# eridgd/WCT-TF

Hardware: NVIDIA B200
Metric: 512x512 5-level WCT stylised frames/sec (higher is better)
Workload: dtype f32

## Files before the change

wct_tf_b200/_capi.py:

```python
from __future__ import annotations

import ctypes as C
import os

_HERE = os.path.dirname(os.path.abspath(__file__))
LIB_PATH = os.path.join(_HERE, "libwctb200.so")

RELU = 1
CLIP01 = 2
HALO_EDGE = 4
POOL2 = 8
EINVAL, ECUDA, EWS, EDEVICE = -1, -2, -3, -4

_vp, _i, _f, _sz = C.c_void_p, C.c_int, C.c_float, C.c_size_t

SIGNATURES = {
    "wctb200_abi_version": (_i, []),
    "wctb200_last_error": (C.c_char_p, []),
    "wctb200_check_device": (_i, [_vp]),
    "wctb200_act_bytes": (_sz, [_i, _i, _i, _i]),
    "wctb200_act_from_f32": (_i, [_vp, _i, _i, _i, _i, _vp, _vp]),
    "wctb200_act_to_f32": (_i, [_vp, _i, _i, _i, _i, _vp, _vp]),
    "wctb200_image_u8_to_f32": (_i, [_vp, _sz, _vp, _vp]),
    "wctb200_image_f32_to_u8": (_i, [_vp, _sz, _vp, _vp]),
    "wctb200_resize_workspace_bytes": (_sz, [_i, _i, _i, _i, _i, _i, _i]),
    "wctb200_resize_bilinear_u8": (_i, [_vp, _i, _i, _i, _i, _i, _i, _i, _i, _i, _i, _vp, _vp, _sz, _vp]),
    "wctb200_rgb_moments_u8": (_i, [_vp, C.c_longlong, _vp, _vp]),
    "wctb200_coral_apply_u8": (_i, [_vp, C.c_longlong, _vp, _vp, _vp, _vp, _vp, _vp, _vp]),
    "wctb200_conv_weight_bytes": (_sz, [_i, _i, _i]),
    "wctb200_prep_conv_weights": (_i, [_vp, _i, _i, _i, _vp, _vp]),
    "wctb200_prep_conv_weights_up2": (_i, [_vp, _i, _i, _vp, _vp]),
    "wctb200_conv3x3": (_i, [_vp, _i, _i, _i, _i, _vp, _vp, _i, _i, _vp, _vp]),
    "wctb200_conv3x3_up2": (_i, [_vp, _i, _i, _i, _i, _vp, _vp, _i, _i, _vp, _vp]),
    "wctb200_conv3x3_ref": (_i, [_vp, _i, _i, _i, _i, _vp, _vp, _i, _i, _vp, _vp]),
    "wctb200_conv_head": (_i, [_vp, _i, _i, _i, _vp, _vp, _vp, _vp]),
    "wctb200_conv_tail": (_i, [_vp, _i, _i, _i, _i, _vp, _vp, _i, _vp, _vp]),
    "wctb200_maxpool2": (_i, [_vp, _i, _i, _i, _i, _vp, _vp]),
    "wctb200_upsample2": (_i, [_vp, _i, _i, _i, _i, _vp, _vp]),
    "wctb200_wct_workspace_bytes": (_sz, [_i, _i, _i]),
    "wctb200_wct_level": (_i, [_vp, _i, _i, _i, _vp, _i, _i, _i, _i, _f, _f, _f, _f, _i, _vp, _vp, _vp, _sz, _vp]),
    "wctb200_wct_style_state_bytes": (_sz, [_i, _i]),
    "wctb200_wct_style_prepare": (_i, [_vp, _i, _i, _i, _i, _f, _f, _f, _vp, _vp, _sz, _vp]),
    "wctb200_wct_apply": (_i, [_vp, _i, _i, _i, _i, _vp, _i, _f, _f, _f, _f, _i, _vp, _vp, _vp, _sz, _vp]),
    "wctb200_adain_level": (_i, [_vp, _i, _i, _i, _vp, _i, _i, _i, _i, _f, _f, _vp, _vp, _sz, _vp]),
    "wctb200_covariance": (_i, [_vp, _i, _i, _i, _i, _f, _vp, _vp, _vp]),
    "wctb200_jacobi_eigh": (_i, [_vp, _i, _i, _vp, _vp, _vp]),
    "wctb200_style_swap_workspace_bytes": (_sz, [_i, _i, _i, _i, _i, _i, _i]),
    "wctb200_style_swap_level": (_i, [_vp, _i, _i, _vp, _i, _i, _i, _i, _i, _f, _f, _f, _vp, _vp, _vp, _sz, _vp]),
}

DEBUG_SIGNATURES = {
    "wctb200_debug_set_conv_bn": (_i, [_i]),
    "wctb200_debug_set_conv_oversub": (_i, [_i]),
    "wctb200_debug_set_conv_fuse": (_i, [_i]),
    "wctb200_debug_set_jacobi": (_i, [_i, _i]),
    "wctb200_debug_set_jacobi_tolq": (_i, [_f]),
    "wctb200_debug_set_conv_products": (_i, [_i]),
    "wctb200_debug_set_conv_tail_tc": (_i, [_i]),
    "wctb200_debug_set_conv_head_tc": (_i, [_i]),
    "wctb200_debug_set_matfun": (_i, [_i, _i]),
    "wctb200_debug_matfun": (_i, [_vp, _i, _i, _i, _f, _f, _vp, _vp, _vp, _vp]),
    "wctb200_debug_set_cov_stages": (_i, [_i]),
}

_lib = None


class WctB200Error(RuntimeError):
    pass


def load():
    global _lib
    if _lib is not None:
        return _lib
    if not os.path.exists(LIB_PATH):
        raise WctB200Error("%s not found: build it with `python -c 'import __graft_entry__ as g; g.build()'` "
                           "(there is no CPU fallback)" % LIB_PATH)
    lib = C.CDLL(LIB_PATH)
    for table in (SIGNATURES, DEBUG_SIGNATURES):
        for name, (res, args) in table.items():
            fn = getattr(lib, name)
            fn.restype = res
            fn.argtypes = args
    if lib.wctb200_abi_version() != 1:
        raise WctB200Error("libwctb200 ABI version mismatch")
    _lib = lib
    return lib


def check(rc):
    if rc != 0:
        raise WctB200Error("libwctb200 error %d: %s" % (rc, load().wctb200_last_error().decode()))
```

wct_tf_b200/csrc/capi.cu:

```cuda
#include <stdarg.h>
#include <string.h>

#include <map>
#include <mutex>
#include <tuple>

#include "common.cuh"
#include "wctb200_debug.h"

namespace wctb {

static thread_local char t_err[512] = "";

void set_error(const char* fmt, ...) {
    va_list ap;
    va_start(ap, fmt);
    vsnprintf(t_err, sizeof(t_err), fmt, ap);
    va_end(ap);
}
int cuda_fail(cudaError_t e, const char* what) {
    set_error("CUDA error %d (%s) at %s", (int)e, cudaGetErrorString(e), what);
    return WCTB200_ECUDA;
}

// ... 6 lines not shown
    std::lock_guard<std::mutex> lock(mu);
    Entry& e = cache[std::make_tuple(dev, st, slot)];
    if (e.cap < bytes) {
        if (e.p) {
            WCTB_CUDA(cudaStreamSynchronize(st));
            WCTB_CUDA(cudaFree(e.p));
            e.p = nullptr;
            e.cap = 0;
        }
        const size_t cap = bytes + bytes / 8 + 256;
        WCTB_CUDA(cudaMalloc(&e.p, cap));
        e.cap = cap;
    }
    *ptr = e.p;
    return 0;
}

__device__ unsigned int g_device_error = 0;

unsigned int* device_error_word() {
    static unsigned int* ptr[64] = {nullptr};
    int dev = 0;
    cudaGetDevice(&dev);
    if (dev < 0 || dev >= 64) dev = 0;
    if (!ptr[dev]) {
        void* p = nullptr;
        if (cudaGetSymbolAddress(&p, g_device_error) == cudaSuccess) ptr[dev] = static_cast<unsigned int*>(p);
    }
    return ptr[dev];
}

int device_sm_count() {
    static std::atomic<int> sms[64];
    int dev = 0;
    cudaGetDevice(&dev);
    dev &= 63;
    int v = sms[dev].load(std::memory_order_relaxed);
    if (v <= 0) {
        if (cudaDeviceGetAttribute(&v, cudaDevAttrMultiProcessorCount, dev) != cudaSuccess || v <= 0) v = 148;
        sms[dev].store(v, std::memory_order_relaxed);
    }
    return v;
}

int launch_u8_to_f32(const uint8_t*, size_t, float*, cudaStream_t);
int launch_f32_to_u8(const float*, size_t, uint8_t*, cudaStream_t);
size_t resize_workspace_bytes(int N, int Hs, int Ws, int C, int Hd, int Wd, int Wout);
int launch_resize_u8(const uint8_t* src, int N, int Hs, int Ws, int C, int Hd, int Wd, int y0, int x0, int Hout, int Wout,
                     uint8_t* dst, void* ws, size_t ws_bytes, cudaStream_t st);
int launch_rgb_moments(const uint8_t* img, long long npix, unsigned long long* sums, cudaStream_t st);
int launch_coral_apply(const uint8_t* src, long long npix, const double* A, const double* sm, const double* ss, const double* tm,
                       const double* ts, uint8_t* dst, cudaStream_t st);
int launch_act_from_f32(const float*, ActGeom, __half*, cudaStream_t);
int launch_act_to_f32(const __half*, ActGeom, float*, cudaStream_t);
int launch_prep_weights(const float*, int, int, int, __half*, cudaStream_t);
int launch_prep_weights_up2(const float*, int, int, __half*, cudaStream_t);
size_t style_swap_workspace_bytes(int C, int Hc, int Wc, int Hs, int Ws, int P, int S);
int launch_style_swap_level(const __half* content, int Hc, int Wc, const __half* style, int Hs, int Ws, int C, int patch, int stride,
                            float alpha, float eps_cov, float thresh, __half* out, int32_t* k_out, void* ws, size_t ws_bytes,
                            cudaStream_t st);
int launch_conv3x3_ref(const __half*, ActGeom, const float*, const float*, int, int, __half*, cudaStream_t);
int launch_conv_head(const float*, int, int, int, const float*, const float*, __half*, cudaStream_t);
int launch_conv_tail(const __half*, ActGeom, const float*, const float*, int, float*, cudaStream_t);
int launch_maxpool2(const __half*, ActGeom, __half*, cudaStream_t);
int launch_upsample2(const __half*, ActGeom, __half*, cudaStream_t);
size_t wct_workspace_bytes(int, int, int);
int launch_wct_level(const __half*, int, int, int, const __half*, int, int, int, int, float, float, float, float, int,
                     __half*, int32_t*, void*, size_t, cudaStream_t);
int launch_adain_level(const __half*, int, int, int, const __half*, int, int, int, int, float, float, __half*, void*,
                       size_t, cudaStream_t);
size_t wct_style_state_bytes(int, int);
int launch_wct_style_prepare(const __half*, int, int, int, int, float, float, float, void*, void*, size_t, cudaStream_t);
int launch_wct_apply(const __half*, int, int, int, int, const void*, int, float, float, float, float, int, __half*, int32_t*,
                     void*, size_t, cudaStream_t);
int launch_covariance(const __half*, int, int, int, int, float, float*, float*, cudaStream_t);
int launch_jacobi(float*, int, int, float*, int*, cudaStream_t, const int* skip);
int launch_eig_post(const float*, const float*, float*, int, int, float, float, int, float*, float*, int*, cudaStream_t, const int* skip);
extern int g_conv_bn_override;
extern int g_conv_oversub;
extern int g_conv_fuse;
extern int g_conv_products;
extern int g_conv_tail_tc;
extern int g_conv_head_tc;
int launch_matfun_ns(const float* A, int C, int count, int n_first, float thresh, float eps_eig, float* out, int* ok, int* kcount,
                     cudaStream_t st, float* info);
extern int g_matfun;
extern int g_matfun_max_it;
extern int g_cov_max_stages;
int set_jacobi_tolq(float v);
extern int g_jacobi_lg;
extern int g_jacobi_stagger;

static bool geom_ok(int N, int H, int W, int C) {
    return N >= 1 && H >= 2 && W >= 2 && C >= 8 && C % 8 == 0 &&
           (long long)N * (2ll * H + 2) * (2ll * W + 2) * (C / 8) < (1ll << 32) && (long long)H * W < (1ll << 31);
}

}

using namespace wctb;

#define ST(s) static_cast<cudaStream_t>(s)
#define HP(p) static_cast<__half*>(p)
#define HCP(p) static_cast<const __half*>(p)

extern "C" {

int wctb200_abi_version(void) { return WCTB200_ABI_VERSION; }
const char* wctb200_last_error(void) { return t_err; }

int wctb200_check_device(void* stream) {
    WCTB_CUDA(cudaStreamSynchronize(ST(stream)));
    unsigned int* w = device_error_word();
    if (!w) {
        set_error("device error word unavailable (no CUDA device?)");
        return WCTB200_ECUDA;
    }
    unsigned int v = 0;
    WCTB_CUDA(cudaMemcpy(&v, w, sizeof(v), cudaMemcpyDeviceToHost));
    if (v != 0) {
        unsigned int zero = 0;
        cudaMemcpy(w, &zero, sizeof(zero), cudaMemcpyHostToDevice);
        set_error("device-side pipeline time-out, code 0x%x (0x1xx producer wait, 0x2xx MMA wait, 0x3xx epilogue wait)", v);
        return WCTB200_EDEVICE;
    }
    return 0;
}

size_t wctb200_act_bytes(int N, int H, int W, int C) {
    if (!geom_ok(N, H, W, C)) return 0;
    ActGeom g(N, H, W, C);
    return (size_t)g.plane * 2 * sizeof(__half);
}

int wctb200_act_from_f32(const float* nhwc, int N, int H, int W, int C, void* act, void* stream) {
    WCTB_REQUIRE(geom_ok(N, H, W, C) && nhwc && act, "act_from_f32: bad arguments");
    return launch_act_from_f32(nhwc, ActGeom(N, H, W, C), HP(act), ST(stream));
}
int wctb200_act_to_f32(const void* act, int N, int H, int W, int C, float* nhwc, void* stream) {
    WCTB_REQUIRE(geom_ok(N, H, W, C) && nhwc && act, "act_to_f32: bad arguments");
    return launch_act_to_f32(HCP(act), ActGeom(N, H, W, C), nhwc, ST(stream));
}

int wctb200_image_u8_to_f32(const uint8_t* img, size_t count, float* out, void* stream) {
    WCTB_REQUIRE(img && out, "image_u8_to_f32: null pointer");
    if (count == 0) return 0;
    return launch_u8_to_f32(img, count, out, ST(stream));
}
int wctb200_image_f32_to_u8(const float* img, size_t count, uint8_t* out, void* stream) {
    WCTB_REQUIRE(img && out, "image_f32_to_u8: null pointer");
    if (count == 0) return 0;
    return launch_f32_to_u8(img, count, out, ST(stream));
}

static bool resize_args_ok(int N, int Hs, int Ws, int C, int Hd, int Wd) {
    return N >= 1 && Hs >= 1 && Ws >= 1 && C >= 1 && C <= 4 && Hd >= 1 && Wd >= 1 && Hs <= (1 << 15) && Ws <= (1 << 15) &&
           Hd <= (1 << 15) && Wd <= (1 << 15);
}
size_t wctb200_resize_workspace_bytes(int N, int Hs, int Ws, int C, int Hd, int Wd, int Wout) {
    if (!resize_args_ok(N, Hs, Ws, C, Hd, Wd) || Wout < 1 || Wout > Wd) return 0;
    return resize_workspace_bytes(N, Hs, Ws, C, Hd, Wd, Wout);
}
int wctb200_resize_bilinear_u8(const uint8_t* src, int N, int Hs, int Ws, int C, int Hd, int Wd, int y0, int x0, int Hout,
                               int Wout, uint8_t* dst, void* ws, size_t ws_bytes, void* stream) {
    WCTB_REQUIRE(src && dst && ws, "resize_bilinear_u8: null pointer");
    WCTB_REQUIRE(resize_args_ok(N, Hs, Ws, C, Hd, Wd), "resize_bilinear_u8: bad geometry N=%d %dx%dx%d -> %dx%d", N, Hs, Ws, C, Hd, Wd);
// ... 90 lines not shown
                      void* ws, size_t ws_bytes, void* stream) {
    WCTB_REQUIRE(content && state && out && ws, "wct_apply: null pointer");
    WCTB_REQUIRE(geom_ok(Nc, Hc, Wc, C), "wct_apply: bad geometry");
    return launch_wct_apply(HCP(content), Nc, Hc, Wc, C, state, Ns, alpha, eps_cov, eps_eig, thresh, readd_content_mean,
                            HP(out), k_out, ws, ws_bytes, ST(stream));
}
int wctb200_adain_level(const void* content, int Nc, int Hc, int Wc, const void* style, int Ns, int Hs, int Ws, int C,
                        float alpha, float eps, void* out, void* ws, size_t ws_bytes, void* stream) {
    WCTB_REQUIRE(content && style && out && ws, "adain_level: null pointer");
    WCTB_REQUIRE(geom_ok(Nc, Hc, Wc, C) && geom_ok(Ns, Hs, Ws, C), "adain_level: bad geometry");
    return launch_adain_level(HCP(content), Nc, Hc, Wc, HCP(style), Ns, Hs, Ws, C, alpha, eps, HP(out), ws, ws_bytes,
                              ST(stream));
}

int wctb200_covariance(const void* act, int N, int H, int W, int C, float eps_cov, float* mean, float* cov, void* stream) {
    WCTB_REQUIRE(act && mean && cov && geom_ok(N, H, W, C), "covariance: bad arguments");
    return launch_covariance(HCP(act), N, H, W, C, eps_cov, mean, cov, ST(stream));
}

int wctb200_jacobi_eigh(float* a, int C, int count, float* sigma, int32_t* sweeps, void* stream) {
    WCTB_REQUIRE(a && sigma && count >= 1, "jacobi_eigh: bad arguments");
    WCTB_REQUIRE(C == 64 || C == 128 || C == 256 || C == 512, "jacobi_eigh: C=%d not in {64,128,256,512}", C);
    const size_t nmat = (size_t)count * C * C;
    float* scratch = nullptr;
    {
        int rc0 = scratch_alloc(reinterpret_cast<void**>(&scratch), ((size_t)count * 16 + nmat + (size_t)count * C) * sizeof(float), ST(stream), 2);
        if (rc0) return rc0;
    }
    float* conv = scratch;
    float* a0 = scratch + (size_t)count * 16;
    float* lam = a0 + nmat;
    cudaError_t ce = cudaMemcpyAsync(a0, a, nmat * sizeof(float), cudaMemcpyDeviceToDevice, ST(stream));
    int rc = ce == cudaSuccess ? launch_jacobi(a, C, count, conv, sweeps, ST(stream), nullptr) : cuda_fail(ce, "cudaMemcpyAsync");
    if (!rc) rc = launch_eig_post(a, a0, lam, C, count, 0.f, 0.f, count, sigma, nullptr, nullptr, ST(stream), nullptr);
    return rc;
}

size_t wctb200_style_swap_workspace_bytes(int C, int Hc, int Wc, int Hs, int Ws, int patch, int stride) {
    if (!geom_ok(1, Hc, Wc, C) || !geom_ok(1, Hs, Ws, C) || patch < 1 || patch > 16 || stride < 1 || stride > 16 || Hc < patch ||
        Wc < patch || Hs < patch || Ws < patch)
        return 0;
    return style_swap_workspace_bytes(C, Hc, Wc, Hs, Ws, patch, stride);
}
int wctb200_style_swap_level(const void* content, int Hc, int Wc, const void* style, int Hs, int Ws, int C, int patch, int stride,
                             float alpha, float eps_cov, float thresh, void* out, int32_t* k_out, void* ws, size_t ws_bytes,
                             void* stream) {
    WCTB_REQUIRE(content && style && out && ws, "style_swap_level: null pointer");
    WCTB_REQUIRE(geom_ok(1, Hc, Wc, C) && geom_ok(1, Hs, Ws, C), "style_swap_level: bad geometry");
    return launch_style_swap_level(HCP(content), Hc, Wc, HCP(style), Hs, Ws, C, patch, stride, alpha, eps_cov, thresh, HP(out), k_out, ws,
                                   ws_bytes, ST(stream));
}
int wctb200_debug_set_conv_bn(int bn) {
    g_conv_bn_override = bn;
    return 0;
}
int wctb200_debug_set_conv_oversub(int k) {
    g_conv_oversub = k < 1 ? 1 : (k > 16 ? 16 : k);
    return g_conv_oversub;
}
int wctb200_debug_set_conv_fuse(int mode) {
    g_conv_fuse = mode < 0 ? -1 : (mode ? 1 : 0);
    return g_conv_fuse;
}
int wctb200_debug_set_jacobi_tolq(float tolq) { return set_jacobi_tolq(tolq); }
int wctb200_debug_set_cov_stages(int n) {
    if (n >= 1 && n <= 12) g_cov_max_stages = n;
    return g_cov_max_stages;
}
int wctb200_debug_matfun(const float* A, int C, int count, int n_first, float thresh, float eps_eig, float* out, int* ok,
                         float* info, void* stream) {
    WCTB_REQUIRE(A && out && ok && count >= 1 && n_first >= 0 && n_first <= count, "debug_matfun: bad arguments");
    const int rc = launch_matfun_ns(A, C, count, n_first, thresh, eps_eig, out, ok, nullptr, ST(stream), info);
    return rc < 0 ? rc : 0;
}
int wctb200_debug_set_matfun(int mode, int max_it) {
    if (mode == 0 || mode == 1) g_matfun = mode;
    if (max_it >= 1 && max_it <= 64) g_matfun_max_it = max_it;
    return g_matfun;
}
int wctb200_debug_set_conv_head_tc(int on) {
    if (on == 0 || on == 1) g_conv_head_tc = on;
    return g_conv_head_tc;
}
int wctb200_debug_set_conv_tail_tc(int on) {
    if (on == 0 || on == 1) g_conv_tail_tc = on;
    return g_conv_tail_tc;
}
int wctb200_debug_set_conv_products(int n) {
    if (n >= 1 && n <= 3) g_conv_products = n;
    return g_conv_products;
}

int wctb200_debug_set_jacobi(int lg_groups, int stagger_cycles) {
    if (lg_groups <= 4) g_jacobi_lg = lg_groups < 0 ? -1 : lg_groups;
    g_jacobi_stagger = stagger_cycles < 0 ? -1 : stagger_cycles;
    return g_jacobi_lg;
}

}
```

wct_tf_b200/csrc/common.cuh:

```cuda
#pragma once

#include <cuda.h>
#include <cuda_fp16.h>
#include <cuda_runtime.h>
#include <stdint.h>
#include <stdio.h>

#include <atomic>

#include "../../include/wctb200.h"

namespace wctb {

void set_error(const char* fmt, ...);
int cuda_fail(cudaError_t e, const char* what);
unsigned int* device_error_word();

#define WCTB_CUDA(call)                                        \
    do {                                                       \
        cudaError_t _e = (call);                               \
        if (_e != cudaSuccess) return ::wctb::cuda_fail(_e, #call); \
    } while (0)

#define WCTB_CHECK_LAUNCH(name)                                \
// ... 203 lines not shown
__device__ __forceinline__ bool mbar_try_wait(uint64_t* bar, uint32_t parity) {
    uint32_t ok;
    asm volatile(
        "{\n\t.reg .pred p;\n\t"
#ifdef WCTB_MBAR_TEST_WAIT
        "mbarrier.test_wait.parity.shared::cta.b64 p, [%1], %2;\n\t"
#else
        "mbarrier.try_wait.parity.shared::cta.b64 p, [%1], %2;\n\t"
#endif
        "selp.u32 %0, 1, 0, p;\n\t}"
        : "=r"(ok)
        : "r"(smem_u32(bar)), "r"(parity)
        : "memory");
    return ok != 0;
}
__device__ __forceinline__ unsigned long long globaltimer_ns() {
    unsigned long long t;
    asm volatile("mov.u64 %0, %globaltimer;" : "=l"(t));
    return t;
}
__device__ __forceinline__ void mbar_wait(uint64_t* bar, uint32_t parity, volatile int* abort_flag,
                                          unsigned int* err_word, unsigned int code) {
    if (mbar_try_wait(bar, parity)) return;
    const long long t0 = clock64();
    for (unsigned int it = 1;; ++it) {
        if (mbar_try_wait(bar, parity)) return;
        if ((it & 255u) == 0u) {
            if (*abort_flag) return;
            if (*reinterpret_cast<volatile unsigned int*>(err_word)) { *abort_flag = 1; return; }
            if (clock64() - t0 > 4000000000ll) break;
        }
    }
    *abort_flag = 1;
    atomicExch(err_word, code);
}

__device__ __forceinline__ void tma_prefetch_desc(const void* map) {
    asm volatile("prefetch.tensormap [%0];" ::"l"(reinterpret_cast<uint64_t>(map)) : "memory");
}
__device__ __forceinline__ void tma_load_3d(void* smem_dst, const void* map, uint64_t* bar, int c0, int c1, int c2) {
    asm volatile(
        "cp.async.bulk.tensor.3d.shared::cluster.global.mbarrier::complete_tx::bytes [%0], [%1, {%3, %4, %5}], [%2];"
        ::"r"(smem_u32(smem_dst)), "l"(reinterpret_cast<uint64_t>(map)), "r"(smem_u32(bar)), "r"(c0), "r"(c1), "r"(c2)
        : "memory");
}

__device__ __forceinline__ void tc_fence_before() { asm volatile("tcgen05.fence::before_thread_sync;" ::: "memory"); }
__device__ __forceinline__ void tc_fence_after() { asm volatile("tcgen05.fence::after_thread_sync;" ::: "memory"); }

__device__ __forceinline__ void tmem_alloc(uint32_t* smem_slot, uint32_t ncols) {
    asm volatile("tcgen05.alloc.cta_group::1.sync.aligned.shared::cta.b32 [%0], %1;" ::"r"(smem_u32(smem_slot)), "r"(ncols)
                 : "memory");
    asm volatile("tcgen05.relinquish_alloc_permit.cta_group::1.sync.aligned;" ::: "memory");
}
__device__ __forceinline__ void tmem_dealloc(uint32_t taddr, uint32_t ncols) {
    asm volatile("tcgen05.dealloc.cta_group::1.sync.aligned.b32 %0, %1;" ::"r"(taddr), "r"(ncols) : "memory");
}
__device__ __forceinline__ void umma_f16(uint32_t tmem_d, uint64_t desc_a, uint64_t desc_b, uint32_t idesc,
                                         uint32_t accumulate) {
    asm volatile(
        "{\n\t.reg .pred p;\n\t"
        "setp.ne.b32 p, %4, 0;\n\t"
        "tcgen05.mma.cta_group::1.kind::f16 [%0], %1, %2, %3, p;\n\t}"
        ::"r"(tmem_d), "l"(desc_a), "l"(desc_b), "r"(idesc), "r"(accumulate)
        : "memory");
}
__device__ __forceinline__ void umma_commit(uint64_t* bar) {
    asm volatile("tcgen05.commit.cta_group::1.mbarrier::arrive::one.shared::cluster.b64 [%0];" ::"r"(smem_u32(bar))
                 : "memory");
}
__device__ __forceinline__ void tmem_ld32(uint32_t taddr, uint32_t* r) {
    asm volatile(
        "tcgen05.ld.sync.aligned.32x32b.x32.b32 "
        "{%0, %1, %2, %3, %4, %5, %6, %7, %8, %9, %10, %11, %12, %13, %14, %15, "
        "%16, %17, %18, %19, %20, %21, %22, %23, %24, %25, %26, %27, %28, %29, %30, %31}, [%32];"
        : "=r"(r[0]), "=r"(r[1]), "=r"(r[2]), "=r"(r[3]), "=r"(r[4]), "=r"(r[5]), "=r"(r[6]), "=r"(r[7]), "=r"(r[8]),
          "=r"(r[9]), "=r"(r[10]), "=r"(r[11]), "=r"(r[12]), "=r"(r[13]), "=r"(r[14]), "=r"(r[15]), "=r"(r[16]),
          "=r"(r[17]), "=r"(r[18]), "=r"(r[19]), "=r"(r[20]), "=r"(r[21]), "=r"(r[22]), "=r"(r[23]), "=r"(r[24]),
          "=r"(r[25]), "=r"(r[26]), "=r"(r[27]), "=r"(r[28]), "=r"(r[29]), "=r"(r[30]), "=r"(r[31])
        : "r"(taddr)
        : "memory");
}
__device__ __forceinline__ void tmem_ld_wait() { asm volatile("tcgen05.wait::ld.sync.aligned;" ::: "memory"); }

__device__ __forceinline__ uint64_t umma_desc_sw128(uint32_t smem_addr) {
    uint64_t d = 0;
    d |= (uint64_t)((smem_addr >> 4) & 0x3FFF);
    d |= (uint64_t)1 << 16;
    d |= (uint64_t)(1024 >> 4) << 32;
    d |= (uint64_t)1 << 46;
    d |= (uint64_t)2 << 61;
    return d;
}
__host__ __device__ constexpr uint32_t umma_idesc_f16(int M, int N) {
    return (1u << 4)
           | (0u << 7) | (0u << 10)
           | (0u << 15) | (0u << 16)
           | ((uint32_t)(N >> 3) << 17)
           | ((uint32_t)(M >> 4) << 24);
}
__device__ __forceinline__ uint64_t umma_desc_mn_sw128(uint32_t smem_addr) {
    uint64_t d = 0;
    d |= (uint64_t)((smem_addr >> 4) & 0x3FFF);
    d |= (uint64_t)((8192 >> 4) & 0x3FFF) << 16;
    d |= (uint64_t)((1024 >> 4) & 0x3FFF) << 32;
    d |= (uint64_t)1 << 46;
    d |= (uint64_t)2 << 61;
    return d;
}
__host__ __device__ constexpr uint32_t umma_idesc_f16_mn(int M, int N) {
    return (1u << 4) | (1u << 15) | (1u << 16) | ((uint32_t)(N >> 3) << 17) | ((uint32_t)(M >> 4) << 24);
}
__device__ __forceinline__ void tmem_ld16(uint32_t taddr, uint32_t* r) {
    asm volatile(
        "tcgen05.ld.sync.aligned.32x32b.x16.b32 "
        "{%0, %1, %2, %3, %4, %5, %6, %7, %8, %9, %10, %11, %12, %13, %14, %15}, [%16];"
        : "=r"(r[0]), "=r"(r[1]), "=r"(r[2]), "=r"(r[3]), "=r"(r[4]), "=r"(r[5]), "=r"(r[6]), "=r"(r[7]), "=r"(r[8]),
          "=r"(r[9]), "=r"(r[10]), "=r"(r[11]), "=r"(r[12]), "=r"(r[13]), "=r"(r[14]), "=r"(r[15])
        : "r"(taddr)
        : "memory");
}
#endif

int scratch_alloc(void** ptr, size_t bytes, cudaStream_t st, int slot);

enum ConvMode { CONV_3X3 = 0, CONV_APPLY = 1, CONV_UP2 = 2, CONV_TAPS = 3 };
int launch_conv_tc(int mode, const __half* in, int N, int H, int W, int Cin, const __half* w_split, int nsets,
                   const float* wscale, const float* bias, int Cout, int flags, __half* out, cudaStream_t st, int kw = 3);
static inline const float* weight_scale_ptr(const __half* w_split, int taps_total, int Cin, int Cout) {
    return reinterpret_cast<const float*>(w_split + (size_t)2 * taps_total * Cin * Cout);
}

}
```

wct_tf_b200/csrc/conv_tc.cu:

```cuda
#include "common.cuh"

namespace wctb {

extern int g_conv_bn_override;

struct ConvParams {
    int N, H, W, Cin, Cout, Hp, Wp;
    long long P;
    int mode;
    int taps;
    int kw;
    int products;
    int per_image;
    int pool;
    int pool_tx, pool_ho;
    int nsets;
    int tiles_per_image;
    int flags;
    const float* bias;
    const float* wscale;
    __half* out;
    unsigned int* err;
};

template <int BN, bool FUSE_>
struct Conv2Cfg {
    static constexpr int BM = 128;
    static constexpr int BK = 64;
    static constexpr int A_BYTES = BM * BK * 2;
    static constexpr int B_BYTES = BN * BK * 2;
    static constexpr int STAGE_BYTES = 2 * A_BYTES + 2 * B_BYTES;
    static constexpr int STAGES = BN == 64 ? 4 : (BN == 128 ? 3 : 2);
    static constexpr bool FUSE = FUSE_ && BN <= 128;
    static constexpr int ACC_COLS = FUSE ? 2 * BN : BN;
    static constexpr int NBUF = 512 / ACC_COLS >= 4 ? 4 : 2;
    static constexpr int TMEM_COLS = NBUF * ACC_COLS;
    static constexpr int CH = 4;
    static constexpr int EPI_WARPS = BN == 256 ? 8 : 4;
    static constexpr int THREADS = 64 + 32 * EPI_WARPS;
    static constexpr int NACC = BN / (EPI_WARPS / 4);
    static constexpr int AUX_BYTES = 256 + BN * 4;
    static constexpr int STG_BYTES = BN <= 128 ? 4 * 8192 : 0;
    static constexpr int SMEM_BYTES = STAGES * STAGE_BYTES + AUX_BYTES + STG_BYTES + 1024;
};

struct TileCoord {
    long long p0, p_end;
    int n0, set;
    int cls;
};

__device__ __forceinline__ TileCoord tile_coord(const ConvParams& p, int tile, int n_tiles, int BN) {
    TileCoord t;
    const int nt = tile % n_tiles;
    int mt = tile / n_tiles;
    const long long HpWp = (long long)p.Hp * p.Wp;
    t.n0 = nt * BN;
    t.cls = 0;
    if (p.pool) {
        const int t_ = mt % p.pool_tx;
        const int r_ = mt / p.pool_tx;
        const int i_ = r_ % p.pool_ho;
        const int img = r_ / p.pool_ho;
        t.p0 = img * HpWp + (long long)(2 * i_ + 1) * p.Wp + 1 + 64 * t_;
        t.p_end = p.P;
        t.set = 0;
        t.cls = t_;
    } else if (p.mode == CONV_UP2) {
        t.cls = mt & 3;
        mt >>= 2;
        t.p0 = (long long)mt * 128;
        t.p_end = p.P;
        t.set = t.cls;
    } else if (p.per_image) {
        const int img = mt / p.tiles_per_image;
        const int r = mt - img * p.tiles_per_image;
        t.p0 = img * HpWp + (long long)r * 128;
        t.p_end = (img + 1) * HpWp;
        t.set = p.nsets > 1 ? img : 0;
    } else {
        t.p0 = (long long)mt * 128;
        t.p_end = p.P;
        t.set = 0;
    }
    return t;
}

template <int BN, bool FUSE_>
__global__ void __launch_bounds__(Conv2Cfg<BN, FUSE_>::THREADS, 1)
conv_tc2_kernel(const __grid_constant__ CUtensorMap mapA, const __grid_constant__ CUtensorMap mapB,
                const __grid_constant__ CUtensorMap mapA64, const ConvParams p, const int total_tiles, const int n_tiles) {
    using Cfg = Conv2Cfg<BN, FUSE_>;
    extern __shared__ uint8_t smem_raw[];
    uint8_t* smem = smem_raw + ((1024u - (smem_u32(smem_raw) & 1023u)) & 1023u);
    uint8_t* aux = smem + Cfg::STAGES * Cfg::STAGE_BYTES;
    uint64_t* full = reinterpret_cast<uint64_t*>(aux);
    uint64_t* empty = full + Cfg::STAGES;
    uint64_t* tfull = empty + Cfg::STAGES;
    uint64_t* tempty = tfull + Cfg::NBUF;
    uint32_t* tmem_slot = reinterpret_cast<uint32_t*>(tempty + Cfg::NBUF);
// ... 190 lines not shown
#pragma unroll
                    for (int h = 0; h < 2; ++h) {
                        const float a0 = acc[h * NH + c0], a1 = acc[h * NH + c0 + 8];
                        const float mine = lp ? a1 : a0;
                        const float other = lp ? a0 : a1;
                        mh[h] = fmaxf(mine, __shfl_xor_sync(0xffffffffu, other, 1));
                    }
                    keep[k] = hv ? mh[1] : mh[0];
                    send[k] = hv ? mh[0] : mh[1];
                }
                uint8_t* stg_all = aux + Cfg::AUX_BYTES;
                {
                    float* xb = reinterpret_cast<float*>(stg_all + e * 8192) + lane;
#pragma unroll
                    for (int k = 0; k < Q; ++k) xb[k * 32] = send[k];
                }
                asm volatile("bar.sync 1, %0;" ::"r"(ETHREADS) : "memory");
                {
                    const float* pb = reinterpret_cast<const float*>(stg_all + (e ^ 2) * 8192) + lane;
#pragma unroll
                    for (int k = 0; k < Q; ++k) keep[k] = fmaxf(keep[k], pb[k * 32]);
                }
                const int xe = x & ~1;
                if (xe < p.W && yy0 - 1 < p.H && !*abort_flag) {
                    const int yo = (yy0 - 1) >> 1, xo = xe >> 1;
                    const int flags = halo_flags(go, yo, xo);
                    const unsigned int ppos = (n * (unsigned int)go.Hp + (unsigned int)(yo + 1)) * (unsigned int)go.Wp + (unsigned int)(xo + 1);
                    const int cb = colbase + hv * NH + lp * 8;
#pragma unroll
                    for (int q = 0; q < Q / 8; ++q) {
                        float v[8];
#pragma unroll
                        for (int j = 0; j < 8; ++j) {
                            const float t = fmaf(keep[q * 8 + j], wsc, sbias[cb + q * 16 + j]);
                            v[j] = relu ? fmaxf(t, 0.f) : t;
                        }
                        Half8 hi, lo;
                        split8(v, hi, lo);
                        store8_at(p.out, go, ppos, flags, tc.n0 + cb + q * 16, hi, lo);
                    }
                }
                continue;
            }
            const unsigned int pos = (unsigned int)tc.p0 + (unsigned int)(g * 32 + lane);
            int flags = -1;
            unsigned int ppos = 0;
            if (pos < (unsigned int)tc.p_end) {
                const unsigned int hpwp = (unsigned int)(p.Hp * p.Wp);
                const unsigned int n = pos / hpwp;
                const unsigned int r = pos - n * hpwp;
                const int yy = (int)(r / (unsigned int)p.Wp);
                const int xx = (int)(r - (unsigned int)yy * (unsigned int)p.Wp);
                if (yy >= 1 && yy <= p.H && xx >= 1 && xx <= p.W && !*abort_flag) {
                    int y = yy - 1, x = xx - 1;
                    if (up2) { y = 2 * y + (tc.cls >> 1); x = 2 * x + (tc.cls & 1); }
                    flags = halo_flags(go, y, x);
                    ppos = ((unsigned int)n * (unsigned int)go.Hp + (unsigned int)(y + 1)) * (unsigned int)go.Wp + (unsigned int)(x + 1);
                }
            }
            if (Cfg::STG_BYTES > 0) {
                uint8_t* stg = aux + Cfg::AUX_BYTES + e * 8192;
                store_tile_rows<Cfg::NACC>(acc, wsc, sbias + colbase, relu, stg, lane, ppos, flags, p.out, go, tc.n0 + colbase);
            } else if (flags >= 0) {
#pragma unroll
                for (int q = 0; q < Cfg::NACC / 8; ++q) {
                    float v[8];
#pragma unroll
                    for (int j = 0; j < 8; ++j) {
                        const float t = fmaf(acc[q * 8 + j], wsc, sbias[colbase + q * 8 + j]);
                        v[j] = relu ? fmaxf(t, 0.f) : t;
                    }
                    Half8 hi, lo;
                    split8(v, hi, lo);
                    store8_at(p.out, go, ppos, flags, tc.n0 + colbase + q * 8, hi, lo);
                }
            }
        }
    }
    tc_fence_before();
    __syncthreads();
    if (warp == 1) tmem_dealloc(tmem_base, Cfg::TMEM_COLS);
}

typedef CUresult (*PFN_encodeTiled)(CUtensorMap*, CUtensorMapDataType, cuuint32_t, void*, const cuuint64_t*,
                                    const cuuint64_t*, const cuuint32_t*, const cuuint32_t*, CUtensorMapInterleave,
                                    CUtensorMapSwizzle, CUtensorMapL2promotion, CUtensorMapFloatOOBfill);

static PFN_encodeTiled get_encode() {
    static PFN_encodeTiled fn = nullptr;
    if (!fn) {
        void* ptr = nullptr;
        cudaDriverEntryPointQueryResult q;
        if (cudaGetDriverEntryPoint("cuTensorMapEncodeTiled", &ptr, cudaEnableDefault, &q) == cudaSuccess &&
            q == cudaDriverEntryPointSuccess)
            fn = reinterpret_cast<PFN_encodeTiled>(ptr);
    }
    return fn;
}

int make_tensor_map_3d(CUtensorMap* m, const void* base, uint64_t d0, uint64_t d1, uint64_t d2, uint64_t stride1_bytes,
                    uint64_t stride2_bytes, uint32_t box1) {
    PFN_encodeTiled enc = get_encode();
    if (!enc) {
        set_error("cuTensorMapEncodeTiled entry point not available");
        return WCTB200_ECUDA;
    }
    cuuint64_t dims[3] = {d0, d1, d2};
    cuuint64_t strides[2] = {stride1_bytes, stride2_bytes};
    cuuint32_t box[3] = {64, box1, 1};
    cuuint32_t estr[3] = {1, 1, 1};
    CUresult r = enc(m, CU_TENSOR_MAP_DATA_TYPE_FLOAT16, 3, const_cast<void*>(base), dims, strides, box, estr,
                     CU_TENSOR_MAP_INTERLEAVE_NONE, CU_TENSOR_MAP_SWIZZLE_128B, CU_TENSOR_MAP_L2_PROMOTION_L2_256B,
                     CU_TENSOR_MAP_FLOAT_OOB_FILL_NONE);
    if (r != CUDA_SUCCESS) {
        set_error("cuTensorMapEncodeTiled failed (%d): dims %llu %llu %llu strides %llu %llu box1 %u", (int)r,
                  (unsigned long long)d0, (unsigned long long)d1, (unsigned long long)d2,
                  (unsigned long long)stride1_bytes, (unsigned long long)stride2_bytes, box1);
        return WCTB200_ECUDA;
    }
    return 0;
}

int g_conv_oversub = 4;

template <int BN, bool FUSE_>
static int launch2_bn(const CUtensorMap& mA, const CUtensorMap& mB, const CUtensorMap& mA64, const ConvParams& p, int total_tiles,
                      int n_tiles, cudaStream_t st) {
    using Cfg = Conv2Cfg<BN, FUSE_>;
    WCTB_ENSURE_SMEM((conv_tc2_kernel<BN, FUSE_>), Cfg::SMEM_BYTES);
    int grid = device_sm_count() * (g_conv_oversub > 0 ? g_conv_oversub : 1);
    if (grid > total_tiles) grid = total_tiles;
    conv_tc2_kernel<BN, FUSE_><<<grid, Cfg::THREADS, Cfg::SMEM_BYTES, st>>>(mA, mB, mA64, p, total_tiles, n_tiles);
    WCTB_CHECK_LAUNCH("conv_tc2_kernel");
    return 0;
}

int g_conv_products = 3;
int g_conv_fuse = -1;
int g_conv_bn_override = 0;

int launch_conv_tc(int mode, const __half* in, int N, int H, int W, int Cin, const __half* w_split, int nsets,
                   const float* wscale, const float* bias, int Cout, int flags, __half* out, cudaStream_t st, int kw) {
    WCTB_REQUIRE(N >= 1 && H >= 2 && W >= 2, "conv: bad geometry N=%d H=%d W=%d", N, H, W);
    WCTB_REQUIRE(Cin % 64 == 0 && Cout % 64 == 0 && Cin >= 64 && Cout >= 64, "conv: Cin=%d Cout=%d must be multiples of 64", Cin, Cout);
    WCTB_REQUIRE(mode == CONV_3X3 || mode == CONV_APPLY || mode == CONV_UP2 || mode == CONV_TAPS, "conv: bad mode %d", mode);
    WCTB_REQUIRE(mode != CONV_TAPS || (kw >= 1 && kw <= 16), "conv: bad filter width %d", kw);
    WCTB_REQUIRE(nsets == 1 || (mode == CONV_APPLY && nsets == N), "conv: nsets must be 1 (or N in apply mode)");
    ActGeom gi(N, H, W, Cin);
    WCTB_REQUIRE(gi.P < (1ll << 31) - 4096, "conv: too many padded positions (%lld)", gi.P);
    WCTB_REQUIRE(mode != CONV_UP2 || ActGeom(N, 2 * H, 2 * W, Cout).P < (1ll << 31), "conv: too many output positions");
    const int taps = mode == CONV_3X3 ? 9 : (mode == CONV_UP2 ? 4 : (mode == CONV_TAPS ? kw * kw : 1));
    const int wsets = mode == CONV_UP2 ? 4 : nsets;

    const bool pool = (flags & WCTB200_POOL2) != 0;
    WCTB_REQUIRE(!pool || (mode == CONV_3X3 && (H + 1) / 2 >= 2 && (W + 1) / 2 >= 2), "conv: POOL2 needs the 3x3 mode and a pooled output >= 2x2");
    int BN = Cout % 128 == 0 ? 128 : 64;
    if (g_conv_bn_override && Cout % g_conv_bn_override == 0) BN = g_conv_bn_override;
    if (pool && BN > 128) BN = 128;

    CUtensorMap mA, mB;
    int rc = make_tensor_map_3d(&mA, in, (uint64_t)Cin, (uint64_t)gi.P, 2, (uint64_t)Cin * 2, (uint64_t)gi.plane * 2, 128);
    if (rc) return rc;
    const uint64_t K = (uint64_t)taps * Cin;
    rc = make_tensor_map_3d(&mB, w_split, K, (uint64_t)Cout, (uint64_t)2 * wsets, K * 2, K * Cout * 2, (uint32_t)BN);
    if (rc) return rc;
    CUtensorMap mA64 = mA;
    if (pool) {
        rc = make_tensor_map_3d(&mA64, in, (uint64_t)Cin, (uint64_t)gi.P, 2, (uint64_t)Cin * 2, (uint64_t)gi.plane * 2, 64);
        if (rc) return rc;
    }

    ConvParams p;
    p.N = N; p.H = H; p.W = W; p.Cin = Cin; p.Cout = Cout; p.Hp = gi.Hp; p.Wp = gi.Wp; p.P = gi.P;
    p.mode = mode;
    p.taps = taps;
    p.kw = kw;
    p.products = (mode == CONV_3X3 || mode == CONV_UP2) ? g_conv_products : 3;
    p.nsets = nsets;
    p.per_image = nsets > 1 ? 1 : 0;
    p.tiles_per_image = cdiv((long long)gi.Hp * gi.Wp, 128);
    p.pool = pool ? 1 : 0;
    p.pool_tx = cdiv(W, 64);
    p.pool_ho = (H + 1) / 2;
    p.flags = flags;
    p.bias = bias;
    p.wscale = wscale;
    p.out = out;
    p.err = device_error_word();
    const int m_tiles = pool ? N * p.pool_ho * p.pool_tx : (p.per_image ? N * p.tiles_per_image : cdiv(gi.P, 128));
    const int n_tiles = Cout / BN;
    const int total = m_tiles * n_tiles * (mode == CONV_UP2 ? 4 : 1);
    switch (BN) {
        case 64: return g_conv_fuse == 0 ? launch2_bn<64, false>(mA, mB, mA64, p, total, n_tiles, st)
                                         : launch2_bn<64, true>(mA, mB, mA64, p, total, n_tiles, st);
        case 128: return (g_conv_fuse == 1 || (g_conv_fuse < 0 && (long long)taps * Cin >= 9 * 256))
                             ? launch2_bn<128, true>(mA, mB, mA64, p, total, n_tiles, st)
                             : launch2_bn<128, false>(mA, mB, mA64, p, total, n_tiles, st);
        default: return launch2_bn<256, false>(mA, mB, mA64, p, total, n_tiles, st);
    }
}

}
```

wct_tf_b200/csrc/wctb200_debug.h:

```cpp
#ifndef WCTB200_DEBUG_H
#define WCTB200_DEBUG_H
#include "../../include/wctb200.h"
#ifdef __cplusplus
extern "C" {
#endif
WCTB200_API int wctb200_debug_set_conv_bn(int bn);
WCTB200_API int wctb200_debug_set_conv_oversub(int k);
WCTB200_API int wctb200_debug_set_conv_fuse(int mode);
WCTB200_API int wctb200_debug_set_jacobi(int lg_groups, int stagger_cycles);
WCTB200_API int wctb200_debug_set_jacobi_tolq(float tolq);
WCTB200_API int wctb200_debug_set_cov_stages(int n);
WCTB200_API int wctb200_debug_set_conv_products(int n);
WCTB200_API int wctb200_debug_set_conv_tail_tc(int on);
WCTB200_API int wctb200_debug_set_matfun(int mode, int max_it);
WCTB200_API int wctb200_debug_matfun(const float* A, int C, int count, int n_first, float thresh, float eps_eig, float* out, int* ok,
                                     float* info, void* stream);
WCTB200_API int wctb200_debug_set_conv_head_tc(int on);
#ifdef __cplusplus
}
#endif
#endif
```

Baseline: 272.7.

## Add row-strip conv kernel reusing A tiles across three ky taps

Adds a new tcgen05 conv kernel for 64-to-64 channel 3x3 convolutions. It processes horizontal strips of rows and loads each input row once per kx/k-slice, then multiplies it against the three ky weight slices into rotating TMEM accumulators. Epilogue warps sum the partial rows in TMEM. This cuts A-tile loads by roughly a factor of three versus the per-tile implicit GEMM. In exchange it adds halo-row overhead per strip, a heuristic for strip height, and more complex TMEM bookkeeping with extra TMEM load/store traffic. The path is on by default for Cin=Cout=64.

```diff
diff --git a/wct_tf_b200/_capi.py b/wct_tf_b200/_capi.py
--- a/wct_tf_b200/_capi.py
+++ b/wct_tf_b200/_capi.py
@@ -58,6 +58,8 @@
     "wctb200_debug_set_conv_products": (_i, [_i]),
     "wctb200_debug_set_conv_tail_tc": (_i, [_i]),
     "wctb200_debug_set_conv_head_tc": (_i, [_i]),
+    "wctb200_debug_set_conv_rows": (_i, [_i]),
+    "wctb200_debug_set_conv_rows_strip": (_i, [_i]),
     "wctb200_debug_set_matfun": (_i, [_i, _i]),
     "wctb200_debug_matfun": (_i, [_vp, _i, _i, _i, _f, _f, _vp, _vp, _vp, _vp]),
     "wctb200_debug_set_cov_stages": (_i, [_i]),
diff --git a/wct_tf_b200/csrc/capi.cu b/wct_tf_b200/csrc/capi.cu
--- a/wct_tf_b200/csrc/capi.cu
+++ b/wct_tf_b200/csrc/capi.cu
@@ -112,6 +112,8 @@
 extern int g_conv_products;
 extern int g_conv_tail_tc;
 extern int g_conv_head_tc;
+extern int g_conv_rows;
+extern int g_conv_rows_strip;
 int launch_matfun_ns(const float* A, int C, int count, int n_first, float thresh, float eps_eig, float* out, int* ok, int* kcount,
                      cudaStream_t st, float* info);
 extern int g_matfun;
@@ -368,6 +370,14 @@
     if (on == 0 || on == 1) g_conv_head_tc = on;
     return g_conv_head_tc;
 }
+int wctb200_debug_set_conv_rows(int mode) {
+    if (mode >= 0 && mode <= 2) g_conv_rows = mode;
+    return g_conv_rows;
+}
+int wctb200_debug_set_conv_rows_strip(int rows) {
+    if (rows == 0 || (rows >= 2 && rows <= 64 && rows % 2 == 0)) g_conv_rows_strip = rows;
+    return g_conv_rows_strip;
+}
 int wctb200_debug_set_conv_tail_tc(int on) {
     if (on == 0 || on == 1) g_conv_tail_tc = on;
     return g_conv_tail_tc;
diff --git a/wct_tf_b200/csrc/common.cuh b/wct_tf_b200/csrc/common.cuh
--- a/wct_tf_b200/csrc/common.cuh
+++ b/wct_tf_b200/csrc/common.cuh
@@ -309,6 +309,18 @@
         : "memory");
 }
 __device__ __forceinline__ void tmem_ld_wait() { asm volatile("tcgen05.wait::ld.sync.aligned;" ::: "memory"); }
+__device__ __forceinline__ void tmem_st32(uint32_t taddr, const float* v) {
+    asm volatile(
+        "tcgen05.st.sync.aligned.32x32b.x32.b32 [%0], "
+        "{%1, %2, %3, %4, %5, %6, %7, %8, %9, %10, %11, %12, %13, %14, %15, %16, "
+        "%17, %18, %19, %20, %21, %22, %23, %24, %25, %26, %27, %28, %29, %30, %31, %32};"
+        ::"r"(taddr), "f"(v[0]), "f"(v[1]), "f"(v[2]), "f"(v[3]), "f"(v[4]), "f"(v[5]), "f"(v[6]), "f"(v[7]), "f"(v[8]),
+          "f"(v[9]), "f"(v[10]), "f"(v[11]), "f"(v[12]), "f"(v[13]), "f"(v[14]), "f"(v[15]), "f"(v[16]), "f"(v[17]),
+          "f"(v[18]), "f"(v[19]), "f"(v[20]), "f"(v[21]), "f"(v[22]), "f"(v[23]), "f"(v[24]), "f"(v[25]), "f"(v[26]),
+          "f"(v[27]), "f"(v[28]), "f"(v[29]), "f"(v[30]), "f"(v[31])
+        : "memory");
+}
+__device__ __forceinline__ void tmem_st_wait() { asm volatile("tcgen05.wait::st.sync.aligned;" ::: "memory"); }
 
 __device__ __forceinline__ uint64_t umma_desc_sw128(uint32_t smem_addr) {
     uint64_t d = 0;
diff --git a/wct_tf_b200/csrc/conv_tc.cu b/wct_tf_b200/csrc/conv_tc.cu
--- a/wct_tf_b200/csrc/conv_tc.cu
+++ b/wct_tf_b200/csrc/conv_tc.cu
@@ -16,6 +16,7 @@
     int pool_tx, pool_ho;
     int nsets;
     int tiles_per_image;
+    int strip_rows, strip_segs, strips_per_image;
     int flags;
     const float* bias;
     const float* wscale;
@@ -372,6 +373,291 @@
     if (warp == 1) tmem_dealloc(tmem_base, Cfg::TMEM_COLS);
 }
 
+struct ConvRowsCfg {
+    static constexpr int BM = 128;
+    static constexpr int BK = 64;
+    static constexpr int A_BYTES = BM * BK * 2;
+    static constexpr int WB_BYTES = 64 * BK * 2;
+    static constexpr int STAGE_BYTES = 2 * A_BYTES + 6 * WB_BYTES;
+    static constexpr int STAGES = 2;
+    static constexpr int GROUP_COLS = 256;
+    static constexpr int TMEM_COLS = 512;
+    static constexpr int EPI_WARPS = 4;
+    static constexpr int THREADS = 64 + 32 * EPI_WARPS;
+    static constexpr int AUX_BYTES = 256 + 64 * 4;
+    static constexpr int STG_BYTES = 4 * 8192;
+    static constexpr int SMEM_BYTES = STAGES * STAGE_BYTES + AUX_BYTES + STG_BYTES + 1024;
+};
+
+struct StripCoord {
+    int img, y0, rows, seg;
+};
+
+__device__ __forceinline__ StripCoord strip_coord(const ConvParams& p, int t) {
+    StripCoord s;
+    s.seg = t % p.strip_segs;
+    const int r = t / p.strip_segs;
+    const int rs = r % p.strips_per_image;
+    s.img = r / p.strips_per_image;
+    s.y0 = rs * p.strip_rows;
+    s.rows = min(p.strip_rows, p.H - s.y0);
+    return s;
+}
+
+__device__ __forceinline__ void rows_span(int i, int rows, int& first, int& count) {
+    const int j0 = max(0, i - 2), j1 = min(i, rows - 1);
+    first = j0 % 3;
+    count = j1 - j0 + 1;
+    if (first + count > 3) {
+        first = 0;
+        count = 3;
+    }
+}
+
+__device__ __forceinline__ void rows_store_pooled(float (&v)[64], const ConvParams& p, const ActGeom& go, const StripCoord& s,
+                                                  int y, int g, int lane, float wsc, const float* sbias, bool relu,
+                                                  volatile int* abort_flag) {
+    const int x = 128 * s.seg + g * 32 + lane;
+    if (x >= p.W) {
+        const float ninf = __int_as_float(0xff800000);
+#pragma unroll
+        for (int c = 0; c < 64; ++c) v[c] = ninf;
+    }
+    const int lp = lane & 1;
+    float keep[32];
+#pragma unroll
+    for (int blk = 0; blk < 4; ++blk) {
+#pragma unroll
+        for (int k = 0; k < 8; ++k) {
+            const float a0 = v[blk * 16 + k], a1 = v[blk * 16 + 8 + k];
+            const float mine = lp ? a1 : a0;
+            const float other = lp ? a0 : a1;
+            keep[blk * 8 + k] = fmaxf(mine, __shfl_xor_sync(0xffffffffu, other, 1));
+        }
+    }
+    const int xe = x & ~1;
+    if (xe < p.W && !*abort_flag) {
+        const int yo = y >> 1, xo = xe >> 1;
+        const int flags = halo_flags(go, yo, xo);
+        const unsigned int ppos = ((unsigned int)s.img * (unsigned int)go.Hp + (unsigned int)(yo + 1)) * (unsigned int)go.Wp +
+                                  (unsigned int)(xo + 1);
+#pragma unroll
+        for (int blk = 0; blk < 4; ++blk) {
+            float t8[8];
+#pragma unroll
+            for (int k = 0; k < 8; ++k) {
+                const float t = fmaf(keep[blk * 8 + k], wsc, sbias[blk * 16 + lp * 8 + k]);
+                t8[k] = relu ? fmaxf(t, 0.f) : t;
+            }
+            Half8 hi, lo;
+            split8(t8, hi, lo);
+            store8_at(p.out, go, ppos, flags, blk * 16 + lp * 8, hi, lo);
+        }
+    }
+}
+
+__device__ __forceinline__ void tmem_sum32(uint32_t ta, uint32_t tb, float* d) {
+    uint32_t r0[32], r1[32];
+    tmem_ld32(ta, r0);
+    tmem_ld32(tb, r1);
+    tmem_ld_wait();
+#pragma unroll
+    for (int c = 0; c < 32; ++c) d[c] = __uint_as_float(r0[c]) + __uint_as_float(r1[c]);
+}
+
+__global__ void __launch_bounds__(ConvRowsCfg::THREADS, 1)
+conv_rows_kernel(const __grid_constant__ CUtensorMap mapA, const __grid_constant__ CUtensorMap mapB, const ConvParams p,
+                 const int n_strips) {
+    using Cfg = ConvRowsCfg;
+    extern __shared__ uint8_t smem_raw[];
+    uint8_t* smem = smem_raw + ((1024u - (smem_u32(smem_raw) & 1023u)) & 1023u);
+    uint8_t* aux = smem + Cfg::STAGES * Cfg::STAGE_BYTES;
+    uint64_t* full = reinterpret_cast<uint64_t*>(aux);
+    uint64_t* empty = full + Cfg::STAGES;
+    uint64_t* tfull = empty + Cfg::STAGES;
+    uint64_t* tempty = tfull + 2;
+    uint32_t* tmem_slot = reinterpret_cast<uint32_t*>(tempty + 2);
+    volatile int* abort_flag = reinterpret_cast<volatile int*>(tmem_slot + 1);
+    float* sbias = reinterpret_cast<float*>(aux + 256);
+
+    const int warp = threadIdx.x >> 5;
+    const int lane = threadIdx.x & 31;
+    {
+        __shared__ unsigned int s_prev_err;
+        if (threadIdx.x == 0) s_prev_err = *reinterpret_cast<volatile unsigned int*>(p.err);
+        __syncthreads();
+        if (s_prev_err != 0u) return;
+    }
+    if (threadIdx.x == 0) {
+        for (int s = 0; s < Cfg::STAGES; ++s) {
+            mbar_init(&full[s], 1);
+            mbar_init(&empty[s], 1);
+        }
+        for (int b = 0; b < 2; ++b) {
+            mbar_init(&tfull[b], 1);
+            mbar_init(&tempty[b], Cfg::EPI_WARPS);
+        }
+        *abort_flag = 0;
+        fence_barrier_init();
+        tma_prefetch_desc(&mapA);
+        tma_prefetch_desc(&mapB);
+    }
+    if (warp == 1) tmem_alloc(tmem_slot, Cfg::TMEM_COLS);
+    tc_fence_before();
+    __syncthreads();
+    tc_fence_after();
+    const uint32_t tmem_base = *tmem_slot;
+    const int ksl = p.Cin / Cfg::BK;
+
+    if (warp == 0) {
+        if (lane == 0) {
+            uint32_t itg = 0;
+            for (int t = blockIdx.x; t < n_strips; t += gridDim.x) {
+                const StripCoord sc = strip_coord(p, t);
+                for (int i = 0; i < sc.rows + 2; ++i) {
+                    const int row0 = (sc.img * p.Hp + sc.y0 + i) * p.Wp + 128 * sc.seg;
+                    for (int kx = 0; kx < 3; ++kx) {
+                        for (int ks = 0; ks < ksl; ++ks, ++itg) {
+                            const int s = itg % Cfg::STAGES;
+                            const uint32_t ph = (itg / Cfg::STAGES) & 1;
+                            mbar_wait(&empty[s], ph ^ 1u, abort_flag, p.err, 0x100u + s);
+                            uint8_t* st = smem + s * Cfg::STAGE_BYTES;
+                            mbar_arrive_expect_tx(&full[s], Cfg::STAGE_BYTES);
+                            tma_load_3d(st, &mapA, &full[s], ks * Cfg::BK, row0 + kx, 0);
+                            tma_load_3d(st + Cfg::A_BYTES, &mapA, &full[s], ks * Cfg::BK, row0 + kx, 1);
+#pragma unroll
+                            for (int blk = 0; blk < 3; ++blk) {
+                                const int ky = (i + 3 - blk) % 3;
+                                const int kc = (ky * 3 + kx) * p.Cin + ks * Cfg::BK;
+                                tma_load_3d(st + 2 * Cfg::A_BYTES + blk * Cfg::WB_BYTES, &mapB, &full[s], kc, 0, 0);
+                                tma_load_3d(st + 2 * Cfg::A_BYTES + (3 + blk) * Cfg::WB_BYTES, &mapB, &full[s], kc, 0, 1);
+                            }
+                        }
+                    }
+                }
+            }
+        }
+        __syncwarp();
+    } else if (warp == 1) {
+        if (lane == 0) {
+            uint32_t itg = 0, ev = 0;
+            for (int t = blockIdx.x; t < n_strips; t += gridDim.x) {
+                const StripCoord sc = strip_coord(p, t);
+                for (int i = 0; i < sc.rows + 2; ++i, ++ev) {
+                    const int grp = ev & 1;
+                    mbar_wait(&tempty[grp], ((ev >> 1) & 1) ^ 1u, abort_flag, p.err, 0x400u + grp);
+                    tc_fence_after();
+                    int first, count;
+                    rows_span(i, sc.rows, first, count);
+                    const uint32_t idesc = umma_idesc_f16(Cfg::BM, 64 * count);
+                    const uint32_t tacc = tmem_base + (uint32_t)(grp * Cfg::GROUP_COLS + first * 64);
+                    for (int it = 0; it < 3 * ksl; ++it, ++itg) {
+                        const int s = itg % Cfg::STAGES;
+                        const uint32_t ph = (itg / Cfg::STAGES) & 1;
+                        mbar_wait(&full[s], ph, abort_flag, p.err, 0x200u + s);
+                        tc_fence_after();
+                        const uint32_t st = smem_u32(smem + s * Cfg::STAGE_BYTES);
+                        const uint64_t a_hi = umma_desc_sw128(st);
+                        const uint64_t a_lo = umma_desc_sw128(st + Cfg::A_BYTES);
+                        const uint64_t b_hi = umma_desc_sw128(st + 2 * Cfg::A_BYTES + first * Cfg::WB_BYTES);
+                        const uint64_t b_lo = umma_desc_sw128(st + 2 * Cfg::A_BYTES + (3 + first) * Cfg::WB_BYTES);
+#pragma unroll
+                        for (int k = 0; k < Cfg::BK / 16; ++k) {
+                            const uint64_t ko = (uint64_t)(k * 32 >> 4);
+                            umma_f16(tacc, a_hi + ko, b_hi + ko, idesc, (it == 0 && k == 0) ? 0u : 1u);
+                            if (p.products >= 3) umma_f16(tacc, a_lo + ko, b_hi + ko, idesc, 1u);
+                            if (p.products >= 2) umma_f16(tacc, a_hi + ko, b_lo + ko, idesc, 1u);
+                        }
+                        umma_commit(&empty[s]);
+                    }
+                    umma_commit(&tfull[grp]);
+                }
+            }
+        }
+        __syncwarp();
+    } else {
+        const int g = warp & 3;
+        const int e = warp - 2;
+        constexpr int ETHREADS = 32 * Cfg::EPI_WARPS;
+        const int et = threadIdx.x - 64;
+        ActGeom go(p.N, p.pool ? (p.H + 1) / 2 : p.H, p.pool ? (p.W + 1) / 2 : p.W, p.Cout);
+        go.edge = (p.flags & WCTB200_HALO_EDGE) ? 1 : 0;
+        const bool relu = (p.flags & WCTB200_RELU) != 0;
+        const float wsc = p.wscale ? __ldg(p.wscale) : 1.f;
+        for (int i = et; i < 64; i += ETHREADS) sbias[i] = p.bias ? p.bias[i] : 0.f;
+        asm volatile("bar.sync 1, %0;" ::"r"(ETHREADS) : "memory");
+        uint8_t* stg = aux + Cfg::AUX_BYTES + e * 8192;
+        const uint32_t tlane = tmem_base + ((uint32_t)(g * 32) << 16);
+        float pend[64];
+        uint32_t ev = 0;
+        for (int t = blockIdx.x; t < n_strips; t += gridDim.x) {
+            const StripCoord sc = strip_coord(p, t);
+            for (int i = 0; i < sc.rows + 2; ++i, ++ev) {
+                const int grp = ev & 1;
+                mbar_wait(&tfull[grp], (ev >> 1) & 1, abort_flag, p.err, 0x300u + grp);
+                tc_fence_after();
+                const uint32_t tg = tlane + (uint32_t)(grp * Cfg::GROUP_COLS);
+                const int j2 = i - 2, j1 = i - 1, j0 = i;
+                float acc[64];
+                if (j2 >= 0) {
+                    const uint32_t c = tg + (uint32_t)((j2 % 3) * 64), sum = tlane + (uint32_t)(192 + 256 * (j2 & 1));
+                    tmem_sum32(c, sum, acc);
+                    tmem_sum32(c + 32, sum + 32, acc + 32);
+                }
+                if (j1 >= 0 && j1 < sc.rows) {
+                    const uint32_t c = tg + (uint32_t)((j1 % 3) * 64), sum = tlane + (uint32_t)(192 + 256 * (j1 & 1));
+#pragma unroll 1
+                    for (int h = 0; h < 64; h += 32) {
+                        float v[32];
+                        tmem_sum32(c + h, sum + h, v);
+                        tmem_st32(sum + h, v);
+                    }
+                }
+                if (j0 < sc.rows) {
+                    const uint32_t c = tg + (uint32_t)((j0 % 3) * 64), sum = tlane + (uint32_t)(192 + 256 * (j0 & 1));
+#pragma unroll 1
+                    for (int h = 0; h < 64; h += 32) {
+                        uint32_t r[32];
+                        tmem_ld32(c + h, r);
+                        tmem_ld_wait();
+                        tmem_st32(sum + h, reinterpret_cast<const float*>(r));
+                    }
+                }
+                tmem_st_wait();
+                tc_fence_before();
+                __syncwarp();
+                if (lane == 0) mbar_arrive(&tempty[grp]);
+                if (j2 < 0) continue;
+                if (p.pool) {
+                    if ((j2 & 1) == 0) {
+#pragma unroll
+                        for (int c = 0; c < 64; ++c) pend[c] = acc[c];
+                        if (j2 + 1 < sc.rows) continue;
+                    } else {
+#pragma unroll
+                        for (int c = 0; c < 64; ++c) pend[c] = fmaxf(pend[c], acc[c]);
+                    }
+                    rows_store_pooled(pend, p, go, sc, sc.y0 + j2, g, lane, wsc, sbias, relu, abort_flag);
+                    continue;
+                }
+                const int y = sc.y0 + j2;
+                const int x = 128 * sc.seg + g * 32 + lane;
+                int flags = -1;
+                unsigned int ppos = 0;
+                if (x < p.W && !*abort_flag) {
+                    flags = halo_flags(go, y, x);
+                    ppos = ((unsigned int)sc.img * (unsigned int)go.Hp + (unsigned int)(y + 1)) * (unsigned int)go.Wp +
+                           (unsigned int)(x + 1);
+                }
+                store_tile_rows<64>(acc, wsc, sbias, relu, stg, lane, ppos, flags, p.out, go, 0);
+            }
+        }
+    }
+    tc_fence_before();
+    __syncthreads();
+    if (warp == 1) tmem_dealloc(tmem_base, Cfg::TMEM_COLS);
+}
+
 typedef CUresult (*PFN_encodeTiled)(CUtensorMap*, CUtensorMapDataType, cuuint32_t, void*, const cuuint64_t*,
                                     const cuuint64_t*, const cuuint32_t*, const cuuint32_t*, CUtensorMapInterleave,
                                     CUtensorMapSwizzle, CUtensorMapL2promotion, CUtensorMapFloatOOBfill);
@@ -422,6 +708,37 @@
     if (grid > total_tiles) grid = total_tiles;
     conv_tc2_kernel<BN, FUSE_><<<grid, Cfg::THREADS, Cfg::SMEM_BYTES, st>>>(mA, mB, mA64, p, total_tiles, n_tiles);
     WCTB_CHECK_LAUNCH("conv_tc2_kernel");
+    return 0;
+}
+
+int g_conv_rows = 1;
+int g_conv_rows_strip = 0;
+
+static int launch_rows(const CUtensorMap& mA, const CUtensorMap& mB, ConvParams p, cudaStream_t st) {
+    using Cfg = ConvRowsCfg;
+    WCTB_ENSURE_SMEM(conv_rows_kernel, Cfg::SMEM_BYTES);
+    const int sms = device_sm_count();
+    p.strip_segs = cdiv(p.W, 128);
+    int best_r = 2;
+    long long best_cost = -1;
+    for (int r = 2; r <= 64; r += 2) {
+        const long long strips = (long long)p.N * p.strip_segs * cdiv(p.H, r);
+        const long long cost = ((strips + sms - 1) / sms) * (r + 2);
+        if (best_cost < 0 || cost < best_cost) {
+            best_cost = cost;
+            best_r = r;
+        }
+        if (r >= p.H) break;
+    }
+    if (g_conv_rows_strip > 0) best_r = g_conv_rows_strip;
+    p.strip_rows = best_r;
+    p.strips_per_image = cdiv(p.H, best_r);
+    const long long n_strips = (long long)p.N * p.strip_segs * p.strips_per_image;
+    WCTB_REQUIRE(n_strips < (1ll << 30), "conv: too many strips (%lld)", n_strips);
+    int grid = sms * (g_conv_oversub > 0 ? g_conv_oversub : 1);
+    if (grid > n_strips) grid = (int)n_strips;
+    conv_rows_kernel<<<grid, Cfg::THREADS, Cfg::SMEM_BYTES, st>>>(mA, mB, p, (int)n_strips);
+    WCTB_CHECK_LAUNCH("conv_rows_kernel");
     return 0;
 }
 
@@ -477,6 +794,8 @@
     p.wscale = wscale;
     p.out = out;
     p.err = device_error_word();
+    p.strip_rows = p.strip_segs = p.strips_per_image = 0;
+    if (mode == CONV_3X3 && Cout == 64 && ((Cin == 64 && g_conv_rows) || g_conv_rows == 2)) return launch_rows(mA, mB, p, st);
     const int m_tiles = pool ? N * p.pool_ho * p.pool_tx : (p.per_image ? N * p.tiles_per_image : cdiv(gi.P, 128));
     const int n_tiles = Cout / BN;
     const int total = m_tiles * n_tiles * (mode == CONV_UP2 ? 4 : 1);
diff --git a/wct_tf_b200/csrc/wctb200_debug.h b/wct_tf_b200/csrc/wctb200_debug.h
--- a/wct_tf_b200/csrc/wctb200_debug.h
+++ b/wct_tf_b200/csrc/wctb200_debug.h
@@ -16,6 +16,8 @@
 WCTB200_API int wctb200_debug_matfun(const float* A, int C, int count, int n_first, float thresh, float eps_eig, float* out, int* ok,
                                      float* info, void* stream);
 WCTB200_API int wctb200_debug_set_conv_head_tc(int on);
+WCTB200_API int wctb200_debug_set_conv_rows(int mode);
+WCTB200_API int wctb200_debug_set_conv_rows_strip(int rows);
 #ifdef __cplusplus
 }
 #endif
```

Measured after the change: 286.1, median of 6. 4.9% higher.
